# ReillyBova/Global-Illumination

Measured on AMD Instinct MI355X. Metric: Mpixel-samples/sec (and ms/frame) at 1024^2 aa=2, 1M+1M photons, higher is better.
Workload: dtype f64 (shading/geometry), f32 (photon positions)

## Files before the change

global-illumination_amd/csrc/gi_chunk.h:

```cpp
#pragma once
#include "gi_kernels.h"
#include "gi_estimate.h"

namespace gi {

__device__ __forceinline__ float wmaxf(float v) {
#pragma unroll
  for (int o = 32; o > 0; o >>= 1) v = fmaxf(v, __shfl_xor(v, o, 64));
  return v;
}
__device__ __forceinline__ float wminf(float v) {
#pragma unroll
  for (int o = 32; o > 0; o >>= 1) v = fminf(v, __shfl_xor(v, o, 64));
  return v;
}

__device__ __forceinline__ float metric(float qx, float qy, float qz, const float4 &p) {
  return photon_d2(qx, qy, qz, p.x, p.y, p.z);
}

template <int CAPC>
struct Cands {
  float *b;
  __device__ __forceinline__ float4 get(uint32_t s) const {
// ... 107 lines not shown
      sp--;
      node = (int)__builtin_amdgcn_readfirstlane((int)stk[sp]);
    }
  }
  return reads;
}

__device__ __forceinline__ void chunk_load_query(const KnnArgs &a, int64_t chunk, int lane, bool &valid,
                                                 int64_t &qi, float4 &qp) {
  int64_t qs = chunk * 64 + lane;
  valid = qs < a.nq;
  qi = 0;
  qp = make_float4(0.f, 0.f, 0.f, 0.f);
  if (valid) {
    qi = a.perm ? (int64_t)a.perm[a.q0 + qs] : a.q0 + qs;
    qp = a.qpos[qi];
    valid = __float_as_uint(qp.w) != QMETA_NONE;
  }
}

}
```

global-illumination_amd/csrc/gi_ctx.h:

```cpp
#pragma once
#include <hip/hip_runtime.h>
#include <rccl/rccl.h>
#include <mutex>
#include <string>
#include <thread>
#include <vector>
#include "../../include/gi.h"
#include "gi_dbuf.h"
#include "gi_kdbuild.h"
#include "gi_kernels.h"
#include "gi_scene.h"
#include "gi_sort.h"

#pragma GCC visibility push(hidden)
namespace gi_internal {
using namespace gi;

struct HostMap {
  std::vector<gi_photon> storage;
  std::vector<int32_t> perm;
  std::vector<float> pos4;
  std::vector<uint32_t> rgbe;
  std::vector<float> nodes;
  int nleaves = 1, levels = 0;
// ... 59 lines not shown
  std::vector<DBuf> recv, peer_pix;
  KdBuildScratch kdb;
  DBuf kd_ph;
  DBuf ind_cont, ind_ncont;
  DBuf mc_cont, mc_ncont;
  DBuf mc_cont2, mc_ncont2;
  DBuf mc_wstate, mc_wlist, mc_wcount;
  DBuf prim_rgb;
  DBuf d_rays, d_ray_ids;
  std::vector<gi_ray> ray_stage;
  std::vector<uint64_t> id_stage;
  DBuf ind_tab, mc_tab;
  DBuf ind_trows, ind_rows;
  DBuf ind_masks;
  DBuf spawn, npaths, path_off, nmc, mc_off, nind, ind_off, base, pixels, rgbf, rgb8, stats_bak;
  DBuf qpos[2], qshade[2], qkey[2], qout[2];
  DBuf qseg[2];
  KeySortScratch keysort[2];
  DBuf scan_lvl[8], scan_out[8];
  DBuf pcounts, poffs, pbuf;
  DBuf pkeys, pcursor, ptmp;
  DBuf pacc, pglob;
  KeySortScratch psort;
  DBuf feat_samples, feat_planes, dn_rgbf, dn_planes, dn_img[2];
  DBuf vdn_var, vdn_vlum;
  DBuf rad_frame, rad_samples, rad_mean, rad_var;
  DBuf prim_layers, lay_frame, lay_samples;
  DBuf acc_part;
  DBuf tile_err, tile_nmin, tile_mask;
  DBuf rp_prev, rp_cur;
  DBuf tm_in, tm_out;
// ... 189 lines not shown
```

global-illumination_amd/csrc/gi_estimate.h:

```cpp
#pragma once
#include "gi_kernels.h"

namespace gi {

__device__ __forceinline__ float photon_d2(float qx, float qy, float qz, float px, float py, float pz) {
  float dx = qx - px, dy = qy - py, dz = qz - pz;
  return __builtin_fmaf(dz, dz, __builtin_fmaf(dy, dy, __fmul_rn(dx, dx)));
}

static __device__ __noinline__ double pow_call(double x, double y) { return gm::pow(x, y); }

__device__ __forceinline__ C3 rgbe_decode(uint32_t e) {
  uint32_t ee = e >> 24;
  double inv = ee ? ldexp(1.0, (int)ee - 128 - 8) : 0.0;
  return rgb(ee ? (double)(e & 255u) * inv : 0.0, ee ? (double)((e >> 8) & 255u) * inv : 0.0,
             ee ? (double)((e >> 16) & 255u) * inv : 0.0);
}

__device__ __forceinline__ uint32_t photon_dcode(const KnnArgs &a, uint32_t id) {
  return __float_as_uint(a.map.pos4[4 * (int64_t)id + 3]) & 0xffffu;
}
__device__ __forceinline__ void lut_dir(const KnnArgs &a, uint32_t dcode, double &ix, double &iy, double &iz) {
  ix = a.lut[3 * dcode];
  iy = a.lut[3 * dcode + 1];
  iz = a.lut[3 * dcode + 2];
}

__device__ __forceinline__ bool wrong_side(uint32_t sign, double perp) {
  return (sign == 2u && perp < 0) || (sign == 1u && perp > 0);
}

__device__ __forceinline__ C3 disk_term(double perp, uint32_t e) { return rgbe_decode(e) * fabs(perp); }

__device__ __forceinline__ void irradiance_add(uint32_t e, C3 &o) {
  if (e >> 24) o = o + rgbe_decode(e);
}
__device__ __forceinline__ C3 irradiance_finish(C3 o, double maxd2) { return o / (kPi * maxd2); }

struct EstQuery {
  const QShade &sh;
  const DMaterial &m;
  uint32_t sign;
  double N0, N1, N2;
  V E;
  bool spec;
  bool diff_only;
  double c1 = 1.0, c2 = 1.0;

  __device__ __forceinline__ EstQuery(const KnnArgs &a, int64_t qi, float meta_w, double maxd2)
      : sh(a.qshade[qi]), m(a.mats[qmeta_mat(__float_as_uint(meta_w))]) {
    sign = __float_as_uint(meta_w) & 3u;
    N0 = sh.n[0]; N1 = sh.n[1]; N2 = sh.n[2];
    E = ld3(sh.ex);
    spec = (m.flags & MF_SPECULAR) || (m.n < 0);
    diff_only = !spec && isfinite(m.ks[0]) && isfinite(m.ks[1]) && isfinite(m.ks[2]);
    if (a.filter == 1) c1 = 1.0 / (a.fk * sqrt(maxd2));
    else if (a.filter == 2) {
      c1 = pow_call(2.7182818284590452354, -a.fb);
      c2 = 1.0 / (2.0 * maxd2);
    }
  }

  __device__ __forceinline__ double perp(double ix, double iy, double iz) const {
    return N0 * ix + N1 * iy + N2 * iz;
  }
  __device__ __forceinline__ bool wrong_side(double perp) const { return gi::wrong_side(sign, perp); }

  __device__ __forceinline__ C3 disk_term_kd(double perp, uint32_t e) const {
    C3 p = rgbe_decode(e);
// ... 24 lines not shown
      double f = (1.0 - c1 * sqrt(d2));
      p.r *= f; p.g *= f; p.b *= f;
    } else if (a.filter == 2) {
      double w = (1.0 - (1.0 - pow_call(c1, c2 * d2)) / (1.0 - c1));
      p.r *= w; p.g *= w; p.b *= w;
      tw += w;
    }
  }
};

__device__ __forceinline__ C3 est_gen_miss(const KnnArgs &a) {
  if (a.stats) atomicAdd(a.stats + ST_GEN_MISS, 1ull);
  return rgb(__builtin_nan(""), __builtin_nan(""), __builtin_nan(""));
}

__device__ __forceinline__ void est_finish(const KnnArgs &a, int filter, const QShade &sh, int num,
                                           double maxd2, double tw, C3 &o) {
  bool ok = true;
  if (filter == 0 && maxd2 > 0) {
    o = o / (kPi * maxd2);
  } else if (filter == 1 && maxd2 > 0) {
    o = o / ((1.0 - 2.0 / 3.0 / a.fk) * kPi * maxd2);
  } else if (filter == 2 && tw > 0 && maxd2 > 0) {
    o = o * (a.fa * (num / tw) / (kPi * maxd2));
  } else {
    ok = false;
  }
  if (ok) {
    o.r *= sh.w[0]; o.g *= sh.w[1]; o.b *= sh.w[2];
  } else {
    o.r = o.g = o.b = 0;
// ... 13 lines not shown
```

global-illumination_amd/csrc/gi_host.cpp:

```cpp
#include <chrono>
#include <cmath>
#include <functional>
#include "gi_ctx.h"
#include "gi_radiance.h"

namespace gi_internal __attribute__((visibility("hidden"))) {

hipError_t read_stats(gi_ctx *c, unsigned long long *out) {
  std::vector<unsigned long long> all((size_t)ST_STRIPES * ST_COUNT);
  hipError_t e = hipMemcpyAsync(all.data(), c->res.d_stats.p, ST_BYTES, hipMemcpyDeviceToHost, c->stream);
  if (e == hipSuccess) e = hipStreamSynchronize(c->stream);
  for (int i = 0; i < ST_COUNT; i++) {
    out[i] = 0;
    for (int s = 0; s < ST_STRIPES; s++) out[i] += all[(size_t)s * ST_COUNT + i];
  }
  return e;
}
void log_phase_cycles(const gi_ctx *c, const unsigned long long *s) {
  if (!(c->knn_dbg & 16)) return;
  fprintf(stderr, "[gi] k-NN phase cycles (sum over waves):");
  for (int i = 0; i < 16; i++) fprintf(stderr, " %llu", s[ST_PHASE + i]);
  fprintf(stderr, "\n");
}

int knn_general(const std::vector<DMaterial> &mats, int filter, bool every_material) {
  if (filter != 0) return 1;
  for (const DMaterial &m : mats) {
    if (!every_material && !(m.flags & MF_DIFFUSE) && m.max_kd == 0.0) continue;
    const bool spec = (m.flags & MF_SPECULAR) || (m.n < 0);
    if (spec || !std::isfinite(m.ks[0]) || !std::isfinite(m.ks[1]) || !std::isfinite(m.ks[2]))
      return 1;
  }
  return 0;
}

KnnArgs knn_args(gi_ctx *c, int mi) {
  KnnArgs k;
  memset(&k, 0, sizeof k);
  k.map = c->res.dmap[mi].view();
  k.mats = c->res.d_mats.as<DMaterial>();
  k.lut = c->res.d_lut.as<double>();
  const gi_params &P = c->P;
  k.K = mi == GI_MAP_GLOBAL ? P.global_estimate_size : P.caustic_estimate_size;
  double r = mi == GI_MAP_GLOBAL ? P.global_estimate_dist : P.caustic_estimate_dist;
  k.filter = mi == GI_MAP_GLOBAL ? P.global_filter : P.caustic_filter;
  k.r2f = (float)(r * r);
  k.rmax = r;
  k.fa = P.filter_const_a;
// ... 14 lines not shown
int ensure_dk(gi_ctx *c, KnnArgs &k) {
  MapExec &X = c->mx[map_index(k)];
  MapScratch &XS = c->s.map[map_index(k)];
  DevMap &D = c->res.dmap[map_index(k)];
  if (!c->use_dk || D.n == 0 || k.K <= 0) return GI_OK;
  if (int rc = check_kd_shape(c, k.map.nleaves, k.map.levels)) return rc;
  if (D.dk_k != k.K || D.dk_r2 != k.r2f) {
    D.dk_k = -1;
    HIPCHK(c, XS.dk_q.ensure((size_t)D.n * 16));
    HIPCHK(c, D.dk.ensure((size_t)D.n * 4));
    launch_photon_queries(D.pos4.as<float>(), D.n, XS.dk_q.as<float4>(), X.st);
    KnnArgs d = k;
    d.mode = KNN_MODE_DK;
    d.map.dk = nullptr;
    d.qpos = XS.dk_q.as<float4>();
    d.qshade = nullptr;
    d.perm = nullptr;
    d.nq = D.n;
    d.q0 = 0;
    d.out_dk = D.dk.as<float>();
    d.stats = nullptr;
    d.dbg = 0;
    if (!launch_knn_wave(d, c->wave_cap_mul, X.st))
      return fail(c, GI_ERR_ARG, "k-NN bound pass: unsupported estimate size");
    HIPCHK(c, hipGetLastError());
    HIPCHK(c, hipStreamSynchronize(X.st));
    D.dk_k = k.K;
    D.dk_r2 = k.r2f;
  }
  k.map.dk = D.dk.as<float>();
  return GI_OK;
// ... 240 lines not shown
    launch_knn(a, X.st);
    HIPCHK(c, hipGetLastError());
    int rc = knn_end(c, X, ms);
    if (rc) return rc;
  }
  return GI_OK;
}

struct ListRows {
  int64_t nprim;
  const uint64_t *qmask;
  int64_t trows;
  uint32_t qbase;
};

static int knn_list(gi_ctx *c, int mi, const float4 *qpos, const QShade *qshade, int64_t nq,
             double *out, double *ms, const ListRows *rows = nullptr, uint32_t qbase = 0,
             const uint32_t *app_order = nullptr) {
  MapExec &X = c->mx[mi];
  MapScratch &XS = c->s.map[mi];
  KnnArgs k = knn_args(c, mi);
  k.qpos = qpos;
  k.qshade = qshade;
  k.out = out;
  k.nq = nq;
  if (c->P.irradiance_cache && mi == GI_MAP_GLOBAL) {
    c->last_kind[mi] = 9;
    launch_cached(k, X.st);
    HIPCHK(c, hipGetLastError());
    return GI_OK;
  }
  {
    uint32_t *perm = nullptr;
    if (rows && c->row_order && c->key_bits[mi] <= 10) {
      int64_t nv = 0;
      HIPCHK(c, curve_order_rows(qpos, rows->nprim, rows->qmask, rows->trows, rows->qbase, nq,
                                 c->sbmin, c->sbmax, XS.sorter, &perm, &nv, X.st,
                                 c->surf_key, app_order));
// ... 167 lines not shown
                           hipMemcpyDeviceToDevice, c->stream));
  qbase[0] = (uint32_t)(nprim + B.tind);
  qbase[1] = (uint32_t)nprim;
  a.qind_base = nprim;
  a.tiled_skip = c->row_order && c->key_bits[0] <= 10 && !c->P.irradiance_cache && a.ind_qmask &&
                 (a.total_ind > 0 || B.tind == 0);
  for (int attempt = 0; attempt < 3; attempt++) {
    for (int l = 0; l < 2; l++) {
      size_t cap = std::max<size_t>(c->qcap_hint[l], (size_t)qbase[l] + 1024);
      if (attempt == 0) {
        const double per_mc = std::max(2.0, c->mc_app_rate[l]);
        size_t pred = (size_t)qbase[l] + (size_t)(1.25 * per_mc * (double)a.total_mc) + 1024;
        cap = std::max(cap, std::min<size_t>(pred, 0xFFFFFFF0u));
      }
      HIPCHK(c, c->s.qpos[l].ensure(cap * 16));
      HIPCHK(c, c->s.qshade[l].ensure(cap * sizeof(QShade)));
      HIPCHK(c, c->s.qkey[l].ensure(cap * 8));
      a.qpos[l] = c->s.qpos[l].as<float4>();
      a.qshade[l] = c->s.qshade[l].as<QShade>();
      a.qkey[l] = c->s.qkey[l].as<uint64_t>();
      a.qcap[l] = (uint32_t)std::min<size_t>(cap, 0xFFFFFFF0u);
    }
    if (a.split_ind && a.total_ind > 0) {
      uint64_t cap_s = std::min<uint64_t>(B.ind_full, 64 * ((uint64_t)(B.ind_full * c->ind_frac) / 64 + 1));
      HIPCHK(c, c->s.ind_cont.ensure((size_t)IND_QS * cap_s * sizeof(IndCont)));
      a.ind_cap_s = (uint32_t)cap_s;
      a.ind_cont = c->s.ind_cont.as<IndCont>();
      a.ind_ncont = c->s.ind_ncont.as<uint32_t>();
    }
    a.qcount = c->res.qcount.as<uint32_t>();
    HIPCHK(c, hipMemcpyAsync(c->res.qcount.p, qbase, 8, hipMemcpyHostToDevice, c->stream));
    if (!a.tiled_skip && B.tind > (uint64_t)a.total_ind) launch_ind_pad(a, c->stream);
    launch_path(a, c->stream, c->stream2, c->ev_fork, c->ev_join, true,
                B.mwave.rounds > 0 ? &B.mwave : nullptr);
// ... 34 lines not shown
    a.qapp[l] = B.qbase[l];
    a.qout[l] = nullptr;
    if (nq[l]) {
      HIPCHK(c, c->s.qout[l].ensure((size_t)nq[l] * 24));
      a.qout[l] = c->s.qout[l].as<double>();
      if (!c->map_valid[l])
        HIPCHK(c, hipMemsetAsync(c->s.qout[l].p, 0, (size_t)nq[l] * 24, c->stream));
      else
        run[l] = true;
    }
  }
  for (int l = 0; l < 2; l++) {
    if (!run[l]) continue;
    ListRows lr{B.nprim, a.ind_qmask, (int64_t)(B.tind / 64), B.qbase[0]};
    const bool use_rows = l == 0 && a.ind_qmask && (a.total_ind > 0 || B.tind == 0);
    int rc = knn_list(c, l, a.qpos[l], a.qshade[l], nq[l], c->s.qout[l].as<double>(),
                      B.timed ? &B.knn_ms[l] : nullptr, use_rows ? &lr : nullptr, B.qbase[l],
                      a.sslot[l]);
    if (rc) return rc;
  }
  return GI_OK;
}

static int order_appends(gi_ctx *c, RenderArgs &a, Batch &B) {
  const int64_t nprim = B.nprim;
  for (int l = 0; l < 2; l++) {
    HIPCHK(c, c->s.qseg[l].ensure((size_t)(nprim + 1) * 4));
    a.qseg[l] = c->s.qseg[l].as<uint32_t>();
    const int64_t napp = (int64_t)B.nq[l] - (int64_t)B.qbase[l];
    if (napp <= 0) {
      HIPCHK(c, hipMemsetAsync(c->s.qseg[l].p, 0, (size_t)(nprim + 1) * 4, c->stream));
      a.skey[l] = nullptr;
      a.sslot[l] = nullptr;
// ... 499 lines not shown
```

global-illumination_amd/csrc/gi_kernels.h:

```cpp
#pragma once
#include <hip/hip_runtime.h>
#include <stdint.h>
#include "gi_device.h"

namespace gi {

struct gi_photon_dev {
  float pos[3];
  uint32_t rgbe;
  uint16_t dir;
  uint16_t flags;
};
static_assert(sizeof(gi_photon_dev) == 20, "photon record is 20 bytes");

struct gi_ray_dev {
  double org[3], dir[3];
};
static_assert(sizeof(gi_ray_dev) == 48, "ray record is 48 bytes");

struct Spawn {
  double p[3], n[3], v[3];
  double ct, R;
  double base[3];
  int32_t mat, hit;
// ... 32 lines not shown
  uint32_t pslot, j;
  int32_t iter, hint;
  uint32_t pad[2];
};
static_assert(sizeof(McState) == 208 && alignof(McState) == 16,
              "path state record is 13 16-byte words");

struct McWave {
  McState *state;
  uint32_t *list[2];
  uint32_t *count;
  int32_t rounds;
};
constexpr int MC_WAVE_MAX_ROUNDS = 1024;

struct QShade {
  double n[3];
  double ex[3];
  double w[3];
};

enum {
  ST_RAY = 0, ST_SHADOW, ST_MONTE, ST_TRANS, ST_SPEC, ST_INDIRECT, ST_CAUSTIC,
  ST_KNN, ST_KNN_PHOTONS, ST_KNN_VISITED,
  ST_KNN_C, ST_KNN_C_PHOTONS, ST_KNN_C_VISITED,
  ST_GEN_MISS,
  ST_PHASE = 16,
  ST_COUNT = 32
};
enum { ST_KNN_MAP = ST_KNN_C - ST_KNN
};

struct RenderArgs {
  SceneView S;
  Flags F;
// ... 24 lines not shown
  uint32_t ind_cap_s;
  IndCont *mc_cont;
  uint32_t *mc_ncont;
  uint32_t mc_cap_s;
  uint32_t *mc_next;
  int32_t mc_persist_blocks;
  int32_t spp;
  IndCont *mc_cont2;
  uint32_t *mc_ncont2;
  int64_t qind_base;
  const uint32_t *ind_rows;
  int64_t ind_g0;
  uint64_t *ind_qmask;
  uint64_t *ind_bmask;
  float4 *qpos[2];
  QShade *qshade[2];
  uint64_t *qkey[2];
  uint32_t *qcount;
  uint32_t qcap[2];
  uint32_t qapp[2];
  const uint64_t *skey[2];
  const uint32_t *sslot[2];
  uint32_t *qseg[2];
  uint32_t nq[2];
  double *base;
  double *prim_rgb;
  const double *qout[2];
  float *rgbf;
  uint8_t *rgb8;
  unsigned long long *stats;
};
// ... 110 lines not shown
    uint32_t w = (blockIdx.x * blockDim.x + threadIdx.x) >> 6;
    atomicAdd(dst + (size_t)(w & (ST_STRIPES - 1)) * ST_COUNT, (unsigned long long)v);
  }
}

constexpr uint32_t QMETA_NONE = 0xffffffffu;
constexpr uint32_t QMETA_MAT_MASK = 0x03ffffffu;
constexpr int QMETA_MAX_MATS = 1 << 26;
__host__ __device__ __forceinline__ uint32_t qmeta_mat(uint32_t meta) { return (meta >> 2) & QMETA_MAT_MASK; }

enum { KNN_MODE_RADIANCE = 0, KNN_MODE_IRRADIANCE = 1, KNN_MODE_LIST = 2, KNN_MODE_DK = 3 };

struct KnnArgs {
  KdView map;
  const float4 *qpos;
  const QShade *qshade;
  const uint32_t *perm;
  const DMaterial *mats;
  const double *lut;
  int64_t nq;
  int64_t q0;
  int32_t K;
  int32_t filter;
  int32_t mode;
  int32_t stat_off;
  int32_t sel_slack;
  int32_t chunk_minsub;
  int32_t dk_exact;
  int32_t qpl;
  int32_t dbg;
  int32_t general;
  float r2f;
  double rmax;
  double fa, fb, fk;
  double *out;
  int32_t *out_n;
  float *out_maxd2;
  float *out_dk;
  int32_t *out_idx;
  float *out_d2;
  int32_t *list_idx;
  float *list_d2;
  int32_t *list_n;
  uint32_t *fb_list;
  uint32_t *fb_count;
  float *gheap_d2;
  int32_t *gheap_idx;
// ... 81 lines not shown
```

global-illumination_amd/csrc/gi_kernels.hip:

```cpp
#include <hip/hip_runtime.h>
#include <type_traits>
#include "gi.h"
#include "gi_device.h"
#include "gi_kernels.h"
#include "gi_estimate.h"

namespace gi {

constexpr int SCAN_BLOCK = 256, SCAN_ITEMS = 4, SCAN_TILE = SCAN_BLOCK * SCAN_ITEMS;

__global__ __launch_bounds__(SCAN_BLOCK) void scan_tile_kernel(const uint32_t *in, uint32_t *out,
                                                                uint32_t *block_sums, int64_t n) {
  __shared__ uint32_t s[SCAN_BLOCK];
  int64_t base = (int64_t)blockIdx.x * SCAN_TILE + threadIdx.x * SCAN_ITEMS;
  uint32_t v[SCAN_ITEMS];
  uint32_t sum = 0;
#pragma unroll
  for (int i = 0; i < SCAN_ITEMS; i++) {
    int64_t k = base + i;
    v[i] = (k < n) ? in[k] : 0u;
    sum += v[i];
  }
  s[threadIdx.x] = sum;
  __syncthreads();
// ... 196 lines not shown
  uint32_t j;
  C3 base;
  Counts cnt;
  int64_t fixed[2];
  int hint;
  uint32_t qstripe;
  int64_t cont_slot;
};

__device__ __forceinline__ bool keyed_slot(const RenderArgs &a, int list, int64_t slot) {
  return list != 0 || slot < a.qind_base || slot >= a.qind_base + a.tind;
}

__device__ __forceinline__ void put_none(const RenderArgs &a, int list, int64_t slot) {
  if (a.tiled_skip && !keyed_slot(a, list, slot)) return;
  a.qpos[list][slot] = make_float4(0.f, 0.f, 0.f, __uint_as_float(QMETA_NONE));
  if (keyed_slot(a, list, slot)) a.qkey[list][slot] = ~0ull;
}

__device__ __forceinline__ uint32_t wave_take(uint32_t *counter) {
  const uint64_t act = __ballot(1);
  const int lane = (int)(threadIdx.x & 63);
  const int leader = __ffsll((long long)act) - 1;
  uint32_t base = 0;
  if (lane == leader) base = atomicAdd(counter, (uint32_t)__popcll(act));
  base = (uint32_t)__shfl((int)base, leader, 64);
  return base + (uint32_t)__popcll(act & ((1ull << lane) - 1ull));
}

__device__ __forceinline__ void put_query(PathCtx &P, int list, V p, V n, V ex, double ct,
                                          int mat, C3 w) {
// ... 2 lines not shown
  if (P.fixed[list] >= 0) {
    slot = (uint32_t)P.fixed[list];
    P.fixed[list] = -2;
  } else {
    slot = wave_take(&a.qcount[list]);
  }
  uint64_t key = ((uint64_t)P.prim << 32) | ((uint64_t)(P.pslot & 0xffffu) << 16) |
                 (uint64_t)(P.j++ & 0xffffu);
  if (slot >= a.qcap[list]) return;
  uint32_t sign = (ct > 0) ? 1u : ((ct < 0) ? 2u : 0u);
  const double ax = fabs(n.x), ay = fabs(n.y), az = fabs(n.z);
  const bool a0 = ax >= ay && ax >= az, a1 = !a0 && ay >= az;
  const double nw = a0 ? n.x : a1 ? n.y : n.z;
  const uint32_t face = (a0 ? 0u : a1 ? 2u : 4u) + (nw < 0.0 ? 1u : 0u);
  uint32_t meta = sign | ((uint32_t)mat << 2) | (face << 28);
  a.qpos[list][slot] = make_float4((float)p.x, (float)p.y, (float)p.z, __uint_as_float(meta));
  QShade q;
  q.n[0] = n.x; q.n[1] = n.y; q.n[2] = n.z;
  q.ex[0] = ex.x; q.ex[1] = ex.y; q.ex[2] = ex.z;
  q.w[0] = w.r; q.w[1] = w.g; q.w[2] = w.b;
  a.qshade[list][slot] = q;
  if (keyed_slot(a, list, slot)) a.qkey[list][slot] = key;
}

__device__ __forceinline__ void global_query(PathCtx &P, V p, V n, V ex, double ct, int mat, C3 w) {
  put_query(P, 0, p, n, ex, ct, mat, w);
}

template <bool DIFFUSE_ONLY, bool UNIT_TW = false>
__device__ __forceinline__ bool ind_shade(PathCtx &P, const Hit &h, V &org, V &dir, Rng &rng, C3 W,
                                          C3 &tw) {
  const SceneView &S = *P.S;
  const Flags &F = *P.F;
  const DMaterial &m = S.mats[h.mat];
  V view = normalize(h.p - org);
  double ct = dot(h.n, -view);
// ... 274 lines not shown
__global__ __launch_bounds__(64) void ind_tile_rows_kernel(const uint32_t *nind, int64_t nprim,
                                                          uint32_t *rows) {
  const int64_t b = (int64_t)blockIdx.x * 64 + threadIdx.x;
  uint32_t v = b < nprim ? nind[b] : 0u;
#pragma unroll
  for (int o = 32; o > 0; o >>= 1) v = max(v, (uint32_t)__shfl_xor((int)v, o, 64));
  if (threadIdx.x == 0) rows[blockIdx.x] = v;
}

__global__ __launch_bounds__(256) void ind_pad_kernel(RenderArgs a) {
  const int64_t b = (int64_t)blockIdx.x * blockDim.x + threadIdx.x;
  if (b >= ((a.nprim + 63) & ~(int64_t)63)) return;
  const int rows = (int)(a.ind_rows[(b >> 6) + 1] - a.ind_rows[b >> 6]);
  for (int s = b < a.nprim ? (int)a.nind[b] : 0; s < rows; s++) {
    const int64_t sl = a.qind_base + ind_tau(a, b, s);
    a.qpos[0][sl] = make_float4(0.f, 0.f, 0.f, __uint_as_float(QMETA_NONE));
  }
}

__device__ __forceinline__ void path_init(PathCtx &P, const RenderArgs &a, int64_t g, int64_t prim,
                                          int pslot) {
  P.S = &a.S;
  P.F = &a.F;
  P.A = &a;
  P.g = (uint64_t)g;
  P.prim = (uint32_t)prim;
  P.pslot = (uint32_t)pslot;
  P.j = 0;
  P.base = rgb(0, 0, 0);
  Counts z = {0, 0, 0, 0, 0, 0};
  P.cnt = z;
// ... 1211 lines not shown
```

global-illumination_amd/csrc/gi_knn.hip:

```cpp
#include <hip/hip_runtime.h>
#include <cstdlib>
#include "gi_device.h"
#include "gi_kernels.h"
#include "gi_estimate.h"

namespace gi {

__device__ __forceinline__ uint32_t ufirst(uint32_t v) {
  return (uint32_t)__builtin_amdgcn_readfirstlane((int)v);
}
__device__ __forceinline__ float ffirst(float v) {
  return __int_as_float(__builtin_amdgcn_readfirstlane(__float_as_int(v)));
}

__device__ __forceinline__ double wave_sum(double v) {
#pragma unroll
  for (int o = 32; o > 0; o >>= 1) v += __shfl_xor(v, o, 64);
  return v;
}
__device__ __forceinline__ C3 wave_sum(C3 v) { return rgb(wave_sum(v.r), wave_sum(v.g), wave_sum(v.b)); }

__device__ __forceinline__ uint32_t radix_pick(uint32_t *hist, int lane, uint32_t &need) {
  uint32_t c0 = hist[4 * lane], c1 = hist[4 * lane + 1], c2 = hist[4 * lane + 2],
           c3 = hist[4 * lane + 3];
// ... 186 lines not shown
  __shared__ uint64_t buf[CAP];
  __shared__ uint32_t hist[256];
  __shared__ uint32_t stk[64];
  __shared__ float sdist[64];
  const int lane = threadIdx.x;
  const float4 *pos = reinterpret_cast<const float4 *>(a.map.pos4);
  const int L = a.map.nleaves;
  const int64_t N = a.map.n;
  const int K = a.K;
  uint64_t st_q = 0, st_found = 0, st_vis = 0;
  const bool prof = PROF;
  uint64_t pc[6] = {0, 0, 0, 0, 0, 0}, pt = 0, pq = 0;
  for (int64_t qq = blockIdx.x; qq < a.nq; qq += gridDim.x) {
    int64_t qg = a.q0 + qq;
    int64_t qi = a.perm ? (int64_t)a.perm[qg] : qg;
    float4 qp = a.qpos[qi];
    if (__float_as_uint(qp.w) == QMETA_NONE) {
      if (FUSE) {
        if (lane == 0) {
          a.out[3 * qi] = a.out[3 * qi + 1] = a.out[3 * qi + 2] = 0.0;
          if (a.out_n) a.out_n[qi] = 0;
          if (a.out_maxd2) a.out_maxd2[qi] = 0.0f;
        }
      } else if (lane == 0 && a.list_n) {
        a.list_n[qi] = 0;
      }
      continue;
    }
    float qx = ffirst(qp.x), qy = ffirst(qp.y), qz = ffirst(qp.z);
    uint32_t count = 0;
    uint64_t thr = ((uint64_t)__float_as_uint(a.r2f) << 32) + 0x100000000ull;
// ... 572 lines not shown
```

global-illumination_amd/csrc/gi_knn_chunk.hip:

```cpp
#include <hip/hip_runtime.h>
#include <hipcub/hipcub.hpp>
#include <cstdlib>
#include <type_traits>
#include "gi_device.h"
#include "gi_kernels.h"
#include "gi_estimate.h"
#include "gi_chunk.h"

namespace gi {

__device__ __forceinline__ double wmax(double v) {
#pragma unroll
  for (int o = 32; o > 0; o >>= 1) v = fmax(v, __shfl_xor(v, o, 64));
  return v;
}

#ifndef CHUNK_EST_EB
#define CHUNK_EST_EB 4
#endif
#ifndef EST_GROUPS
#define EST_GROUPS 3
#endif

__device__ __forceinline__ float wave_sort(float v, int lane) {
// ... 377 lines not shown
            eg[u] = crgbe[slot];
            lut_dir(a, __float_as_uint(cpos.wbits(slot)) & 0xffffu, lg[u][0], lg[u][1], lg[u][2]);
          }
#pragma unroll
          for (int u = 0; u < EB; u++) {
            if (s0 + u >= num) break;
            double perp = Q.perp(lg[u][0], lg[u][1], lg[u][2]);
            if (Q.wrong_side(perp)) continue;
            o = o + disk_term(perp, eg[u]);
          }
        }
        o = o * kd;
      } else if constexpr (!GEN) {
        o = est_gen_miss(a);
      } else {
        const V E = ld3(Q.sh.ex);
        for (int s = 0; s < num; s++) {
          uint32_t slot = slot_at(s);
          float4 p = cpos.get(slot);
          uint32_t e = crgbe[slot];
          double ix, iy, iz;
          lut_dir(a, __float_as_uint(p.w) & 0xffffu, ix, iy, iz);
          double d2 = (double)metric(qp.x, qp.y, qp.z, p);
          double perp = Q.perp(ix, iy, iz);
          if (Q.wrong_side(perp)) continue;
          C3 t;
          Q.general_term(a, E, ix, iy, iz, perp, e, d2, t, tw);
          o = o + t;
        }
      }
      est_finish(a, a.filter, Q.sh, num, maxd2, tw, o);
// ... 5 lines not shown
template <int CAPC, typename SlotAt, typename PerLane>
__device__ __forceinline__ void chunk_estimate_shared(const KnnArgs &a, int lane, bool col, int64_t qi,
                                                      float4 qp, int num, float km, uint32_t count,
                                                      const Cands<CAPC> &cpos, const uint32_t *crgbe,
                                                      double *tp, SlotAt slot_at, PerLane per_lane) {
  bool shp = false;
  double N0 = 0.0, N1 = 0.0, N2 = 0.0;
  uint32_t sign = 0u;
  const DMaterial *mt = nullptr;
  if (col && num > 0 && a.mode == KNN_MODE_RADIANCE && a.filter == 0 && !(a.dbg & 256)) {
    const uint32_t meta = __float_as_uint(qp.w);
    mt = &a.mats[qmeta_mat(meta)];
    const bool spec = (mt->flags & MF_SPECULAR) || (mt->n < 0);
    shp = !spec && isfinite(mt->ks[0]) && isfinite(mt->ks[1]) && isfinite(mt->ks[2]);
    if (shp) {
      const QShade &sh = a.qshade[qi];
      N0 = sh.n[0]; N1 = sh.n[1]; N2 = sh.n[2];
      sign = meta & 3u;
    }
  }
  uint64_t rem = __ballot(shp);
  int gi = -1, ng = 0;
  int lead[EST_GROUPS];
#pragma unroll
  for (int g = 0; g < EST_GROUPS; g++) {
    lead[g] = 0;
    if (!rem) continue;
    const int L0 = __ffsll((long long)rem) - 1;
    const long long l0 = __shfl(__double_as_longlong(N0), L0, 64);
    const long long l1 = __shfl(__double_as_longlong(N1), L0, 64);
    const long long l2 = __shfl(__double_as_longlong(N2), L0, 64);
// ... 54 lines not shown
          t[u][2] = tp[2 * CAPC + sl[u]];
        }
#pragma unroll
        for (int u = 0; u < EB; u++) {
          if (k0 + u >= num) break;
          o0 += t[u][0]; o1 += t[u][1]; o2 += t[u][2];
        }
      }
    }
  }
  if (gi >= 0) {
    const int K = a.K;
    double maxd2 = (num < K) ? a.rmax * a.rmax : (double)km;
    if (num == K && maxd2 < kEps) maxd2 = kEps;
    C3 o = rgb(o0, o1, o2) * ldc(mt->kd);
    est_finish(a, 0, a.qshade[qi], num, maxd2, 0.0, o);
    est_store(a, qi, num, maxd2, o);
  }
}

__device__ __forceinline__ void chunk_flush_stats(const KnnArgs &a, const ChunkProf &P, uint64_t q,
                                                  uint64_t found, uint64_t vis) {
  if (P.on && a.stats)
    for (int i = 0; i < 10; i++) wave_add(&a.stats[ST_PHASE + i], P.c[i]);
  if (a.stats) {
    wave_add(&a.stats[ST_KNN + a.stat_off], q);
    wave_add(&a.stats[ST_KNN_PHOTONS + a.stat_off], found);
    wave_add(&a.stats[ST_KNN_VISITED + a.stat_off], vis);
  }
}

// ... 548 lines not shown
```

global-illumination_amd/csrc/gi_knn_heap.hip:

```cpp
#include <hip/hip_runtime.h>
#include "gi_device.h"
#include "gi_kernels.h"
#include "gi_estimate.h"

namespace gi {

struct HeapRef {
  float *d2;
  int32_t *idx;
  int stride;
};

__device__ __forceinline__ bool heap_less(float da, int ia, float db, int ib) {
  return da < db || (da == db && ia < ib);
}

__device__ __forceinline__ void heap_push(HeapRef h, int &size, float d, int id) {
  int c = size++;
  while (c > 0) {
    int p = (c - 1) >> 1;
    float pd = h.d2[p * h.stride];
    int pi = h.idx[p * h.stride];
    if (!heap_less(pd, pi, d, id)) break;
    h.d2[c * h.stride] = pd;
// ... 159 lines not shown
    }
  }
  if (a.stats) {
    wave_add(&a.stats[ST_KNN + a.stat_off], nq_done);
    wave_add(&a.stats[ST_KNN_PHOTONS + a.stat_off], nfound_total);
    wave_add(&a.stats[ST_KNN_VISITED + a.stat_off], visited_total);
  }
}

__global__ __launch_bounds__(64) void cached_kernel(KnnArgs a) {
  int64_t q = (int64_t)blockIdx.x * 64 + threadIdx.x;
  uint64_t nq_done = 0;
  if (q < a.nq && __float_as_uint(a.qpos[q].w) != QMETA_NONE) {
    float4 qp = a.qpos[q];
    nq_done = 1;
    const QShade &sh = a.qshade[q];
    uint32_t meta = __float_as_uint(qp.w);
    uint32_t sign = meta & 3u;
    const DMaterial &m = a.mats[qmeta_mat(meta)];
    double N0 = sh.n[0], N1 = sh.n[1], N2 = sh.n[2];
    double out0 = 0, out1 = 0, out2 = 0;
    double closest = 0;
    const KdNode *nodes = reinterpret_cast<const KdNode *>(a.map.nodes);
    const float4 *pos = reinterpret_cast<const float4 *>(a.map.pos4);
    const int L = a.map.nleaves;
    for (int guard = 0; guard < 1 << 20 && a.map.n > 0; guard++) {
      double mn = closest + kEps;
      float min2 = (float)(mn * mn);
      float best2 = a.r2f;
      int best = -1;
      int node = 1;
// ... 22 lines not shown
          float qq = kd_axis_q(__float_as_int(pn.hi.w), qp.x, qp.y, qp.z);
          int near_is_right = (qq - pn.lo.w >= 0.0f) ? 1 : 0;
          if ((node & 1) == near_is_right) break;
          node >>= 1;
        }
        if (node == 1) break;
        node ^= 1;
      }
      closest = sqrt((double)best2);
      if (best < 0) break;
      double ix, iy, iz;
      lut_dir(a, photon_dcode(a, (uint32_t)best), ix, iy, iz);
      double perp = N0 * ix + N1 * iy + N2 * iz;
      if (wrong_side(sign, perp)) continue;
      C3 p = rgbe_decode(a.map.rgbe[best]);
      double ca = sh.ex[0] * -ix + sh.ex[1] * -iy + sh.ex[2] * -iz;
      if (ca < 0) ca = 0;
      double ap = fabs(perp);
      double pw = gm::pow(ca, m.n);
      double p0 = p.r * (ap * m.kd[0] + pw * m.ks[0]);
      double p1 = p.g * (ap * m.kd[1] + pw * m.ks[1]);
      double p2 = p.b * (ap * m.kd[2] + pw * m.ks[2]);
      out0 = p0 * sh.w[0];
      out1 = p1 * sh.w[1];
      out2 = p2 * sh.w[2];
      break;
    }
    a.out[3 * q] = out0;
    a.out[3 * q + 1] = out1;
    a.out[3 * q + 2] = out2;
  }
// ... 16 lines not shown
```

global-illumination_amd/csrc/gi_probe.cpp:

```cpp
#include <cfloat>
#include <cmath>
#include "gi_ctx.h"
#include "gi_radiance.h"

extern "C" {

int gi_radiance_bench(gi_ctx *c, int aa, int w, int h, int warmup, int reps, double *reduce_ms,
                      double *merge_ms, double *noise_ms) {
  if (!c) return GI_ERR_ARG;
  if (aa < 0 || aa > 15 || w <= 0 || h <= 0 || warmup < 0 || reps < 1 || reps > 10000)
    return fail(c, GI_ERR_ARG, "radiance bench: bad size or repetition count");
  const int64_t S = (int64_t)1 << (2 * aa);
  const size_t npix = (size_t)w * h;
  if ((int64_t)npix >= ((int64_t)1 << 31) / S) return fail(c, GI_ERR_ARG, "radiance bench: frame too large");
  DeviceScope dev(c->device);
  std::vector<int32_t> pix(npix * 2);
  for (size_t p = 0; p < npix; p++) {
    pix[2 * p] = (int32_t)(p % w);
    pix[2 * p + 1] = (int32_t)(p / w);
  }
  DBuf prim, pixels, frame, acc, cnt, part;
  hipEvent_t e0 = nullptr, e1 = nullptr;
  const size_t nb = (npix + NOISE_BLOCK - 1) / NOISE_BLOCK;
  auto run = [&]() -> hipError_t {
// ... 149 lines not shown
  if (e1) hipEventDestroy(e1);
  HIPCHK(c, e);
  return GI_OK;
}

int gi_estimate_radiance_batch(gi_ctx *c, int map, int64_t n, const gi_radiance_query *q,
                               double *rgb_out, int32_t *nfound, float *maxd2) {
  if (!c || map < 0 || map > 1 || (n > 0 && (!q || !rgb_out))) return GI_ERR_ARG;
  if (n == 0) return GI_OK;
  for (int64_t i = 1; i < n; i++)
    if (q[i].k != q[0].k || q[i].max_dist != q[0].max_dist || q[i].filter != q[0].filter)
      return fail(c, GI_ERR_ARG, "estimate_size / estimate_dist / filter must be uniform");
  if (n > QMETA_MAX_MATS) return fail(c, GI_ERR_ARG, "at most 2^26 queries per call");
  std::vector<DMaterial> mats(n);
  std::vector<float> qp(4 * n);
  std::vector<QShade> qs(n);
  for (int64_t i = 0; i < n; i++) {
    DMaterial &m = mats[i];
    memset(&m, 0, sizeof m);
    for (int j = 0; j < 3; j++) { m.kd[j] = q[i].kd[j]; m.ks[j] = q[i].ks[j]; }
    m.n = q[i].shininess;
    bool spec = !(m.ks[0] == 0.0 && m.ks[1] == 0.0 && m.ks[2] == 0.0);
    m.flags = spec ? MF_SPECULAR : 0;
    double ct = q[i].cos_theta;
    uint32_t sign = (ct > 0) ? 1u : ((ct < 0) ? 2u : 0u);
    uint32_t meta = sign | ((uint32_t)i << 2);
    qp[4 * i] = (float)q[i].point[0];
    qp[4 * i + 1] = (float)q[i].point[1];
    qp[4 * i + 2] = (float)q[i].point[2];
    memcpy(&qp[4 * i + 3], &meta, 4);
    for (int j = 0; j < 3; j++) {
      qs[i].n[j] = q[i].normal[j];
      qs[i].ex[j] = q[i].exact_bounce[j];
      qs[i].w[j] = 1.0;
    }
  }
  DBuf dm, dq, ds, dout, dn, dmd;
  HIPCHK(c, upload(dm, mats.data(), mats.size() * sizeof(DMaterial), c->stream));
  HIPCHK(c, upload(dq, qp.data(), qp.size() * 4, c->stream));
  HIPCHK(c, upload(ds, qs.data(), qs.size() * sizeof(QShade), c->stream));
  HIPCHK(c, dout.ensure((size_t)n * 24));
  HIPCHK(c, dn.ensure((size_t)n * 4));
  HIPCHK(c, dmd.ensure((size_t)n * 4));
  KnnArgs k = knn_args(c, map);
  k.mats = dm.as<DMaterial>();
  k.K = q[0].k;
  k.filter = q[0].filter;
  k.general = c->knn_general_mode > 0 ? 1 : knn_general(mats, k.filter, true);
  k.r2f = (float)(q[0].max_dist * q[0].max_dist);
  k.rmax = q[0].max_dist;
  k.qpos = dq.as<float4>();
  k.qshade = ds.as<QShade>();
  k.out = dout.as<double>();
  k.out_n = dn.as<int32_t>();
  k.out_maxd2 = dmd.as<float>();
  unsigned long long *miss = c->res.d_stats.as<unsigned long long>() + ST_GEN_MISS;
  for (int pass = 0;; pass++) {
    HIPCHK(c, hipMemsetAsync(miss, 0, 8, c->stream));
    int rc = run_knn(c, k, n, nullptr);
    if (rc) return rc;
    unsigned long long nm = 0;
    HIPCHK(c, hipMemcpyAsync(&nm, miss, 8, hipMemcpyDeviceToHost, c->stream));
    HIPCHK(c, hipStreamSynchronize(c->stream));
    if (nm == 0) break;
    if (pass > 0 || k.general) return fail(c, GI_ERR_STATE, "k-NN estimate: general-form miss");
    k.general = 1;
  }
// ... 34 lines not shown
  HIPCHK(c, hipMemcpyAsync(d2_out, dd.p, (size_t)n * K * 4, hipMemcpyDeviceToHost, c->stream));
  HIPCHK(c, hipMemcpyAsync(nfound, dn.p, (size_t)n * 4, hipMemcpyDeviceToHost, c->stream));
  HIPCHK(c, hipStreamSynchronize(c->stream));
  const auto &perm = c->hmap[map].perm;
  for (size_t i = 0; i < idx.size(); i++) idx_out[i] = idx[i] >= 0 ? perm[idx[i]] : -1;
  return GI_OK;
}

int gi_knn_bench(gi_ctx *c, int map, int64_t n, const double *pts, const double *nrm,
                 const int32_t *mat, int mode, int kernel, int iters, double *ms_out,
                 double *found_out, double *visited_out) {
  if (!c || map < 0 || map > 1 || n <= 0 || !pts || iters <= 0 || mode < 0 || mode > 2)
    return GI_ERR_ARG;
  if (mode == KNN_MODE_RADIANCE && (!nrm || !mat || !c->have_scene))
    return fail(c, GI_ERR_STATE, "radiance mode needs normals, materials and a scene");
  std::vector<float> qp(4 * n, 0.0f);
  std::vector<QShade> qs(n);
  for (int64_t i = 0; i < n; i++) {
    for (int j = 0; j < 3; j++) qp[4 * i + j] = (float)pts[3 * i + j];
    uint32_t meta = mat ? ((uint32_t)std::max(0, mat[i]) << 2) : 0u;
    memcpy(&qp[4 * i + 3], &meta, 4);
    for (int j = 0; j < 3; j++) {
      qs[i].n[j] = nrm ? nrm[3 * i + j] : 0.0;
      qs[i].ex[j] = nrm ? nrm[3 * i + j] : 0.0;
      qs[i].w[j] = 1.0;
    }
  }
  KnnArgs k = knn_args(c, map);
  DBuf dq, ds, dout, di, dd, dn;
  HIPCHK(c, upload(dq, qp.data(), qp.size() * 4, c->stream));
  HIPCHK(c, upload(ds, qs.data(), qs.size() * sizeof(QShade), c->stream));
  HIPCHK(c, dout.ensure((size_t)n * 24));
  k.qpos = dq.as<float4>();
  k.qshade = ds.as<QShade>();
  k.out = dout.as<double>();
  k.mode = mode;
  if (mode == KNN_MODE_LIST) {
    HIPCHK(c, di.ensure((size_t)n * k.K * 4));
    HIPCHK(c, dd.ensure((size_t)n * k.K * 4));
    HIPCHK(c, dn.ensure((size_t)n * 4));
    k.out_idx = di.as<int32_t>();
    k.out_d2 = dd.as<float>();
    k.out_n = dn.as<int32_t>();
  }
  float bmin[3], bmax[3];
  for (int j = 0; j < 3; j++) { bmin[j] = FLT_MAX; bmax[j] = -FLT_MAX; }
  for (int64_t i = 0; i < n; i++)
    for (int j = 0; j < 3; j++) {
      bmin[j] = std::min(bmin[j], qp[4 * i + j]);
// ... 67 lines not shown
```

Measured before the change: 13.87.

## Pack query position, normal and weight into a 64-byte record; split exact-bounce out

Replaces the 72-byte QShade struct and the separate position array read in k-NN kernels with a 64-byte aligned QRec holding position+meta, normal and weight. The exact-bounce vector moves to a side array appended after the records, written and read only for specular materials or when the irradiance cache or general mode needs it. The goal is one cache-line-friendly record fetch per query instead of a float4 load plus a 72-byte struct that straddles lines. In exchange, query emission now writes the position twice (qpos plus qrec) and buffer sizing depends on scene materials.

```diff
diff --git a/global-illumination_amd/csrc/gi_chunk.h b/global-illumination_amd/csrc/gi_chunk.h
--- a/global-illumination_amd/csrc/gi_chunk.h
+++ b/global-illumination_amd/csrc/gi_chunk.h
@@ -145,7 +145,7 @@
   qp = make_float4(0.f, 0.f, 0.f, 0.f);
   if (valid) {
     qi = a.perm ? (int64_t)a.perm[a.q0 + qs] : a.q0 + qs;
-    qp = a.qpos[qi];
+    qp = query_pos(a, qi);
     valid = __float_as_uint(qp.w) != QMETA_NONE;
   }
 }
diff --git a/global-illumination_amd/csrc/gi_ctx.h b/global-illumination_amd/csrc/gi_ctx.h
--- a/global-illumination_amd/csrc/gi_ctx.h
+++ b/global-illumination_amd/csrc/gi_ctx.h
@@ -97,7 +97,7 @@
   DBuf ind_trows, ind_rows;
   DBuf ind_masks;
   DBuf spawn, npaths, path_off, nmc, mc_off, nind, ind_off, base, pixels, rgbf, rgb8, stats_bak;
-  DBuf qpos[2], qshade[2], qkey[2], qout[2];
+  DBuf qpos[2], qrec[2], qkey[2], qout[2];
   DBuf qseg[2];
   KeySortScratch keysort[2];
   DBuf scan_lvl[8], scan_out[8];
diff --git a/global-illumination_amd/csrc/gi_estimate.h b/global-illumination_amd/csrc/gi_estimate.h
--- a/global-illumination_amd/csrc/gi_estimate.h
+++ b/global-illumination_amd/csrc/gi_estimate.h
@@ -37,22 +37,34 @@
 }
 __device__ __forceinline__ C3 irradiance_finish(C3 o, double maxd2) { return o / (kPi * maxd2); }
 
+#ifndef QREC_POS
+#define QREC_POS 1
+#endif
+__device__ __forceinline__ float4 query_pos(const KnnArgs &a, int64_t qi) {
+  if (QREC_POS && a.qrec) return a.qrec[qi].pm;
+  return a.qpos[qi];
+}
+
+__device__ __forceinline__ V est_ex(const KnnArgs &a, int64_t qi, bool spec) {
+  return spec ? ld3(qrec_ex(a.qrec, a.qcap) + 3 * qi) : mk(0.0, 0.0, 0.0);
+}
+
 struct EstQuery {
-  const QShade &sh;
+  const QRec &sh;
   const DMaterial &m;
   uint32_t sign;
   double N0, N1, N2;
+  bool spec;
   V E;
-  bool spec;
   bool diff_only;
   double c1 = 1.0, c2 = 1.0;
 
   __device__ __forceinline__ EstQuery(const KnnArgs &a, int64_t qi, float meta_w, double maxd2)
-      : sh(a.qshade[qi]), m(a.mats[qmeta_mat(__float_as_uint(meta_w))]) {
+      : sh(a.qrec[qi]), m(a.mats[qmeta_mat(__float_as_uint(meta_w))]) {
     sign = __float_as_uint(meta_w) & 3u;
     N0 = sh.n[0]; N1 = sh.n[1]; N2 = sh.n[2];
-    E = ld3(sh.ex);
-    spec = (m.flags & MF_SPECULAR) || (m.n < 0);
+    spec = mat_spec(m);
+    E = est_ex(a, qi, spec);
     diff_only = !spec && isfinite(m.ks[0]) && isfinite(m.ks[1]) && isfinite(m.ks[2]);
     if (a.filter == 1) c1 = 1.0 / (a.fk * sqrt(maxd2));
     else if (a.filter == 2) {
@@ -107,7 +119,7 @@
   return rgb(__builtin_nan(""), __builtin_nan(""), __builtin_nan(""));
 }
 
-__device__ __forceinline__ void est_finish(const KnnArgs &a, int filter, const QShade &sh, int num,
+__device__ __forceinline__ void est_finish(const KnnArgs &a, int filter, const QRec &sh, int num,
                                            double maxd2, double tw, C3 &o) {
   bool ok = true;
   if (filter == 0 && maxd2 > 0) {
diff --git a/global-illumination_amd/csrc/gi_host.cpp b/global-illumination_amd/csrc/gi_host.cpp
--- a/global-illumination_amd/csrc/gi_host.cpp
+++ b/global-illumination_amd/csrc/gi_host.cpp
@@ -32,6 +32,13 @@
       return 1;
   }
   return 0;
+}
+
+static bool need_qex(const gi_ctx *c) {
+  if (c->knn_general_mode > 0 || c->P.irradiance_cache) return true;
+  for (const DMaterial &m : c->scene.mats)
+    if (mat_spec(m)) return true;
+  return false;
 }
 
 KnnArgs knn_args(gi_ctx *c, int mi) {
@@ -76,7 +83,7 @@
     d.mode = KNN_MODE_DK;
     d.map.dk = nullptr;
     d.qpos = XS.dk_q.as<float4>();
-    d.qshade = nullptr;
+    d.qrec = nullptr;
     d.perm = nullptr;
     d.nq = D.n;
     d.q0 = 0;
@@ -347,14 +354,15 @@
   uint32_t qbase;
 };
 
-static int knn_list(gi_ctx *c, int mi, const float4 *qpos, const QShade *qshade, int64_t nq,
-             double *out, double *ms, const ListRows *rows = nullptr, uint32_t qbase = 0,
+static int knn_list(gi_ctx *c, int mi, const float4 *qpos, const QRec *qrec, uint32_t qcap,
+             int64_t nq, double *out, double *ms, const ListRows *rows = nullptr, uint32_t qbase = 0,
              const uint32_t *app_order = nullptr) {
   MapExec &X = c->mx[mi];
   MapScratch &XS = c->s.map[mi];
   KnnArgs k = knn_args(c, mi);
   k.qpos = qpos;
-  k.qshade = qshade;
+  k.qrec = qrec;
+  k.qcap = qcap;
   k.out = out;
   k.nq = nq;
   if (c->P.irradiance_cache && mi == GI_MAP_GLOBAL) {
@@ -552,10 +560,10 @@
         cap = std::max(cap, std::min<size_t>(pred, 0xFFFFFFF0u));
       }
       HIPCHK(c, c->s.qpos[l].ensure(cap * 16));
-      HIPCHK(c, c->s.qshade[l].ensure(cap * sizeof(QShade)));
+      HIPCHK(c, c->s.qrec[l].ensure(cap * (sizeof(QRec) + (need_qex(c) ? QEX_BYTES : 0))));
       HIPCHK(c, c->s.qkey[l].ensure(cap * 8));
       a.qpos[l] = c->s.qpos[l].as<float4>();
-      a.qshade[l] = c->s.qshade[l].as<QShade>();
+      a.qrec[l] = c->s.qrec[l].as<QRec>();
       a.qkey[l] = c->s.qkey[l].as<uint64_t>();
       a.qcap[l] = (uint32_t)std::min<size_t>(cap, 0xFFFFFFF0u);
     }
@@ -620,9 +628,9 @@
     if (!run[l]) continue;
     ListRows lr{B.nprim, a.ind_qmask, (int64_t)(B.tind / 64), B.qbase[0]};
     const bool use_rows = l == 0 && a.ind_qmask && (a.total_ind > 0 || B.tind == 0);
-    int rc = knn_list(c, l, a.qpos[l], a.qshade[l], nq[l], c->s.qout[l].as<double>(),
-                      B.timed ? &B.knn_ms[l] : nullptr, use_rows ? &lr : nullptr, B.qbase[l],
-                      a.sslot[l]);
+    int rc = knn_list(c, l, a.qpos[l], a.qrec[l], need_qex(c) ? a.qcap[l] : 0u, nq[l],
+                      c->s.qout[l].as<double>(), B.timed ? &B.knn_ms[l] : nullptr,
+                      use_rows ? &lr : nullptr, B.qbase[l], a.sslot[l]);
     if (rc) return rc;
   }
   return GI_OK;
diff --git a/global-illumination_amd/csrc/gi_kernels.h b/global-illumination_amd/csrc/gi_kernels.h
--- a/global-illumination_amd/csrc/gi_kernels.h
+++ b/global-illumination_amd/csrc/gi_kernels.h
@@ -1,5 +1,6 @@
 #pragma once
 #include <hip/hip_runtime.h>
+#include <stddef.h>
 #include <stdint.h>
 #include "gi_device.h"
 
@@ -70,11 +71,24 @@
 };
 constexpr int MC_WAVE_MAX_ROUNDS = 1024;
 
-struct QShade {
+struct alignas(64) QRec {
+  float4 pm;
   double n[3];
-  double ex[3];
   double w[3];
 };
+static_assert(sizeof(QRec) == 64 && alignof(QRec) == 64, "query record is one 64-byte half line");
+static_assert(offsetof(QRec, pm) == 0 && offsetof(QRec, n) == 16 && offsetof(QRec, w) == 40,
+              "query record layout");
+constexpr size_t QEX_BYTES = 24;
+__host__ __device__ __forceinline__ bool mat_spec(const DMaterial &m) {
+  return (m.flags & MF_SPECULAR) || (m.n < 0);
+}
+__host__ __device__ __forceinline__ double *qrec_ex(QRec *rec, uint32_t cap) {
+  return reinterpret_cast<double *>(rec + cap);
+}
+__host__ __device__ __forceinline__ const double *qrec_ex(const QRec *rec, uint32_t cap) {
+  return reinterpret_cast<const double *>(rec + cap);
+}
 
 enum {
   ST_RAY = 0, ST_SHADOW, ST_MONTE, ST_TRANS, ST_SPEC, ST_INDIRECT, ST_CAUSTIC,
@@ -129,7 +143,7 @@
   uint64_t *ind_qmask;
   uint64_t *ind_bmask;
   float4 *qpos[2];
-  QShade *qshade[2];
+  QRec *qrec[2];
   uint64_t *qkey[2];
   uint32_t *qcount;
   uint32_t qcap[2];
@@ -270,7 +284,7 @@
 struct KnnArgs {
   KdView map;
   const float4 *qpos;
-  const QShade *qshade;
+  const QRec *qrec;
   const uint32_t *perm;
   const DMaterial *mats;
   const double *lut;
@@ -287,6 +301,7 @@
   int32_t dbg;
   int32_t general;
   float r2f;
+  uint32_t qcap;
   double rmax;
   double fa, fb, fk;
   double *out;
diff --git a/global-illumination_amd/csrc/gi_kernels.hip b/global-illumination_amd/csrc/gi_kernels.hip
--- a/global-illumination_amd/csrc/gi_kernels.hip
+++ b/global-illumination_amd/csrc/gi_kernels.hip
@@ -234,7 +234,9 @@
 
 __device__ __forceinline__ void put_none(const RenderArgs &a, int list, int64_t slot) {
   if (a.tiled_skip && !keyed_slot(a, list, slot)) return;
-  a.qpos[list][slot] = make_float4(0.f, 0.f, 0.f, __uint_as_float(QMETA_NONE));
+  const float4 none = make_float4(0.f, 0.f, 0.f, __uint_as_float(QMETA_NONE));
+  a.qpos[list][slot] = none;
+  a.qrec[list][slot].pm = none;
   if (keyed_slot(a, list, slot)) a.qkey[list][slot] = ~0ull;
 }
 
@@ -267,12 +269,16 @@
   const double nw = a0 ? n.x : a1 ? n.y : n.z;
   const uint32_t face = (a0 ? 0u : a1 ? 2u : 4u) + (nw < 0.0 ? 1u : 0u);
   uint32_t meta = sign | ((uint32_t)mat << 2) | (face << 28);
-  a.qpos[list][slot] = make_float4((float)p.x, (float)p.y, (float)p.z, __uint_as_float(meta));
-  QShade q;
+  QRec q;
+  q.pm = make_float4((float)p.x, (float)p.y, (float)p.z, __uint_as_float(meta));
   q.n[0] = n.x; q.n[1] = n.y; q.n[2] = n.z;
-  q.ex[0] = ex.x; q.ex[1] = ex.y; q.ex[2] = ex.z;
   q.w[0] = w.r; q.w[1] = w.g; q.w[2] = w.b;
-  a.qshade[list][slot] = q;
+  a.qpos[list][slot] = q.pm;
+  a.qrec[list][slot] = q;
+  if (mat_spec(P.S->mats[mat]) || P.F->cache) {
+    double *e = qrec_ex(a.qrec[list], a.qcap[list]) + 3 * (size_t)slot;
+    e[0] = ex.x; e[1] = ex.y; e[2] = ex.z;
+  }
   if (keyed_slot(a, list, slot)) a.qkey[list][slot] = key;
 }
 
@@ -577,7 +583,9 @@
   const int rows = (int)(a.ind_rows[(b >> 6) + 1] - a.ind_rows[b >> 6]);
   for (int s = b < a.nprim ? (int)a.nind[b] : 0; s < rows; s++) {
     const int64_t sl = a.qind_base + ind_tau(a, b, s);
-    a.qpos[0][sl] = make_float4(0.f, 0.f, 0.f, __uint_as_float(QMETA_NONE));
+    const float4 none = make_float4(0.f, 0.f, 0.f, __uint_as_float(QMETA_NONE));
+    a.qpos[0][sl] = none;
+    a.qrec[0][sl].pm = none;
   }
 }
 
diff --git a/global-illumination_amd/csrc/gi_knn.hip b/global-illumination_amd/csrc/gi_knn.hip
--- a/global-illumination_amd/csrc/gi_knn.hip
+++ b/global-illumination_amd/csrc/gi_knn.hip
@@ -224,7 +224,7 @@
   for (int64_t qq = blockIdx.x; qq < a.nq; qq += gridDim.x) {
     int64_t qg = a.q0 + qq;
     int64_t qi = a.perm ? (int64_t)a.perm[qg] : qg;
-    float4 qp = a.qpos[qi];
+    float4 qp = query_pos(a, qi);
     if (__float_as_uint(qp.w) == QMETA_NONE) {
       if (FUSE) {
         if (lane == 0) {
diff --git a/global-illumination_amd/csrc/gi_knn_chunk.hip b/global-illumination_amd/csrc/gi_knn_chunk.hip
--- a/global-illumination_amd/csrc/gi_knn_chunk.hip
+++ b/global-illumination_amd/csrc/gi_knn_chunk.hip
@@ -415,7 +415,7 @@
       } else if constexpr (!GEN) {
         o = est_gen_miss(a);
       } else {
-        const V E = ld3(Q.sh.ex);
+        const V E = est_ex(a, qi, Q.spec);
         for (int s = 0; s < num; s++) {
           uint32_t slot = slot_at(s);
           float4 p = cpos.get(slot);
@@ -451,7 +451,7 @@
     const bool spec = (mt->flags & MF_SPECULAR) || (mt->n < 0);
     shp = !spec && isfinite(mt->ks[0]) && isfinite(mt->ks[1]) && isfinite(mt->ks[2]);
     if (shp) {
-      const QShade &sh = a.qshade[qi];
+      const QRec &sh = a.qrec[qi];
       N0 = sh.n[0]; N1 = sh.n[1]; N2 = sh.n[2];
       sign = meta & 3u;
     }
@@ -536,7 +536,7 @@
     double maxd2 = (num < K) ? a.rmax * a.rmax : (double)km;
     if (num == K && maxd2 < kEps) maxd2 = kEps;
     C3 o = rgb(o0, o1, o2) * ldc(mt->kd);
-    est_finish(a, 0, a.qshade[qi], num, maxd2, 0.0, o);
+    est_finish(a, 0, a.qrec[qi], num, maxd2, 0.0, o);
     est_store(a, qi, num, maxd2, o);
   }
 }
diff --git a/global-illumination_amd/csrc/gi_knn_heap.hip b/global-illumination_amd/csrc/gi_knn_heap.hip
--- a/global-illumination_amd/csrc/gi_knn_heap.hip
+++ b/global-illumination_amd/csrc/gi_knn_heap.hip
@@ -197,7 +197,8 @@
   if (q < a.nq && __float_as_uint(a.qpos[q].w) != QMETA_NONE) {
     float4 qp = a.qpos[q];
     nq_done = 1;
-    const QShade &sh = a.qshade[q];
+    const QRec &sh = a.qrec[q];
+    const double *ex = qrec_ex(a.qrec, a.qcap) + 3 * q;
     uint32_t meta = __float_as_uint(qp.w);
     uint32_t sign = meta & 3u;
     const DMaterial &m = a.mats[qmeta_mat(meta)];
@@ -250,7 +251,7 @@
       double perp = N0 * ix + N1 * iy + N2 * iz;
       if (wrong_side(sign, perp)) continue;
       C3 p = rgbe_decode(a.map.rgbe[best]);
-      double ca = sh.ex[0] * -ix + sh.ex[1] * -iy + sh.ex[2] * -iz;
+      double ca = ex[0] * -ix + ex[1] * -iy + ex[2] * -iz;
       if (ca < 0) ca = 0;
       double ap = fabs(perp);
       double pw = gm::pow(ca, m.n);
diff --git a/global-illumination_amd/csrc/gi_probe.cpp b/global-illumination_amd/csrc/gi_probe.cpp
--- a/global-illumination_amd/csrc/gi_probe.cpp
+++ b/global-illumination_amd/csrc/gi_probe.cpp
@@ -187,7 +187,9 @@
   if (n > QMETA_MAX_MATS) return fail(c, GI_ERR_ARG, "at most 2^26 queries per call");
   std::vector<DMaterial> mats(n);
   std::vector<float> qp(4 * n);
-  std::vector<QShade> qs(n);
+  std::vector<unsigned char> qs((size_t)n * (sizeof(QRec) + QEX_BYTES));
+  QRec *rec = reinterpret_cast<QRec *>(qs.data());
+  double *qex = qrec_ex(rec, (uint32_t)n);
   for (int64_t i = 0; i < n; i++) {
     DMaterial &m = mats[i];
     memset(&m, 0, sizeof m);
@@ -202,16 +204,17 @@
     qp[4 * i + 1] = (float)q[i].point[1];
     qp[4 * i + 2] = (float)q[i].point[2];
     memcpy(&qp[4 * i + 3], &meta, 4);
+    memcpy(&rec[i].pm, &qp[4 * i], 16);
     for (int j = 0; j < 3; j++) {
-      qs[i].n[j] = q[i].normal[j];
-      qs[i].ex[j] = q[i].exact_bounce[j];
-      qs[i].w[j] = 1.0;
+      rec[i].n[j] = q[i].normal[j];
+      qex[3 * i + j] = q[i].exact_bounce[j];
+      rec[i].w[j] = 1.0;
     }
   }
   DBuf dm, dq, ds, dout, dn, dmd;
   HIPCHK(c, upload(dm, mats.data(), mats.size() * sizeof(DMaterial), c->stream));
   HIPCHK(c, upload(dq, qp.data(), qp.size() * 4, c->stream));
-  HIPCHK(c, upload(ds, qs.data(), qs.size() * sizeof(QShade), c->stream));
+  HIPCHK(c, upload(ds, qs.data(), qs.size(), c->stream));
   HIPCHK(c, dout.ensure((size_t)n * 24));
   HIPCHK(c, dn.ensure((size_t)n * 4));
   HIPCHK(c, dmd.ensure((size_t)n * 4));
@@ -223,7 +226,8 @@
   k.r2f = (float)(q[0].max_dist * q[0].max_dist);
   k.rmax = q[0].max_dist;
   k.qpos = dq.as<float4>();
-  k.qshade = ds.as<QShade>();
+  k.qrec = ds.as<QRec>();
+  k.qcap = (uint32_t)n;
   k.out = dout.as<double>();
   k.out_n = dn.as<int32_t>();
   k.out_maxd2 = dmd.as<float>();
@@ -288,25 +292,30 @@
     return GI_ERR_ARG;
   if (mode == KNN_MODE_RADIANCE && (!nrm || !mat || !c->have_scene))
     return fail(c, GI_ERR_STATE, "radiance mode needs normals, materials and a scene");
+  if (n > 0xFFFFFFF0ll) return GI_ERR_ARG;
   std::vector<float> qp(4 * n, 0.0f);
-  std::vector<QShade> qs(n);
+  std::vector<unsigned char> qs((size_t)n * (sizeof(QRec) + QEX_BYTES));
+  QRec *rec = reinterpret_cast<QRec *>(qs.data());
+  double *qex = qrec_ex(rec, (uint32_t)n);
   for (int64_t i = 0; i < n; i++) {
     for (int j = 0; j < 3; j++) qp[4 * i + j] = (float)pts[3 * i + j];
     uint32_t meta = mat ? ((uint32_t)std::max(0, mat[i]) << 2) : 0u;
     memcpy(&qp[4 * i + 3], &meta, 4);
+    memcpy(&rec[i].pm, &qp[4 * i], 16);
     for (int j = 0; j < 3; j++) {
-      qs[i].n[j] = nrm ? nrm[3 * i + j] : 0.0;
-      qs[i].ex[j] = nrm ? nrm[3 * i + j] : 0.0;
-      qs[i].w[j] = 1.0;
+      rec[i].n[j] = nrm ? nrm[3 * i + j] : 0.0;
+      qex[3 * i + j] = nrm ? nrm[3 * i + j] : 0.0;
+      rec[i].w[j] = 1.0;
     }
   }
   KnnArgs k = knn_args(c, map);
   DBuf dq, ds, dout, di, dd, dn;
   HIPCHK(c, upload(dq, qp.data(), qp.size() * 4, c->stream));
-  HIPCHK(c, upload(ds, qs.data(), qs.size() * sizeof(QShade), c->stream));
+  HIPCHK(c, upload(ds, qs.data(), qs.size(), c->stream));
   HIPCHK(c, dout.ensure((size_t)n * 24));
   k.qpos = dq.as<float4>();
-  k.qshade = ds.as<QShade>();
+  k.qrec = ds.as<QRec>();
+  k.qcap = (uint32_t)n;
   k.out = dout.as<double>();
   k.mode = mode;
   if (mode == KNN_MODE_LIST) {
```

Result: no change. 13.97 (median of 6 runs) (+0.7%).
